# NVlabs/latentfusion

Measured on AMD Instinct MI355X. Metric: pose-optim iters/sec (reconstruct+render+backward), 16 views, 128^3 voxels, higher is better.
Workload: dtype f32

## Files before the change

### latentfusion_amd/csrc/conv_wino.hip

```cpp
#include "lf_common.h"
#ifndef WINO_ABL
#define WINO_ABL 0
#endif
#ifndef WINO_PJ_ABL
#define WINO_PJ_ABL 0
#endif
#ifndef WINO_PL
#define WINO_PL 2
#endif
#ifndef WINO_PM
#define WINO_PM 1
#endif
#ifndef WINO_PN
#define WINO_PN 3
#endif

namespace {

constexpr int TZw = 2, TYw = 8, TXw = 16;
constexpr int HZw = TZw + 2, HYw = TYw + 2, HXw = TXw + 2;
constexpr int HALOw = HZw * HYw * HXw;
constexpr int HALFw = 2 * HYw * HXw;
constexpr int HALFBw = HALFw * 64;
constexpr int NSLOTw = (HALFw * 4 + 63) / 64;
constexpr int NITw = (NSLOTw + 3) / 4;
constexpr int BUFw = 2 * HALFBw;
constexpr int PXw = 4 * 8192;
constexpr int LDSw = BUFw + PXw + 1024;

__device__ __forceinline__ void lds_barrier() {
  asm volatile("s_waitcnt lgkmcnt(0)\n\ts_barrier" ::: "memory");
}

__device__ __forceinline__ float quad_sum(float v) {
  const float a = v + __int_as_float(__builtin_amdgcn_update_dpp(0, __float_as_int(v), 0xB1, 0xF, 0xF, true));
  return a + __int_as_float(__builtin_amdgcn_update_dpp(0, __float_as_int(a), 0x4E, 0xF, 0xF, true));
}

__device__ __forceinline__ float fast_rsqrt(float x) {
  const float r = __builtin_amdgcn_rsqf(x);
  return r * (1.5f - 0.5f * x * r * r);
}
__device__ __forceinline__ float fast_rcp(float x) {
  const float r = __builtin_amdgcn_rcpf(x);
  return r * (2.f - x * r);
}

typedef float f32x2 __attribute__((ext_vector_type(2)));
__device__ __forceinline__ f32x4 pk_sub(f32x4 a, f32x4 b) {
  f32x2 lo, hi;
  const f32x2 alo = {a[0], a[1]}, ahi = {a[2], a[3]}, blo = {b[0], b[1]}, bhi = {b[2], b[3]};
  asm("v_pk_add_f32 %0, %1, %2 neg_lo:[0,1] neg_hi:[0,1]" : "=v"(lo) : "v"(alo), "v"(blo));
  asm("v_pk_add_f32 %0, %1, %2 neg_lo:[0,1] neg_hi:[0,1]" : "=v"(hi) : "v"(ahi), "v"(bhi));
  return (f32x4){lo[0], lo[1], hi[0], hi[1]};
}

__device__ __forceinline__ void pk_sub_to(f32x4& a, const f32x4 b, int gate = 0) {
  f32x2 alo = {a[0], a[1]}, ahi = {a[2], a[3]};
  const f32x2 blo = {b[0], b[1]}, bhi = {b[2], b[3]};
  asm("v_pk_add_f32 %0, %0, %1 neg_lo:[0,1] neg_hi:[0,1]" : "+v"(alo) : "v"(blo), "s"(gate));
  asm("v_pk_add_f32 %0, %0, %1 neg_lo:[0,1] neg_hi:[0,1]" : "+v"(ahi) : "v"(bhi), "s"(gate));
  a = (f32x4){alo[0], alo[1], ahi[0], ahi[1]};
}
__device__ __forceinline__ void pk_add_to(f32x4& a, const f32x4 b, int gate = 0) {
  f32x2 alo = {a[0], a[1]}, ahi = {a[2], a[3]};
  const f32x2 blo = {b[0], b[1]}, bhi = {b[2], b[3]};
  asm("v_pk_add_f32 %0, %0, %1" : "+v"(alo) : "v"(blo), "s"(gate));
  asm("v_pk_add_f32 %0, %0, %1" : "+v"(ahi) : "v"(bhi), "s"(gate));
  a = (f32x4){alo[0], alo[1], ahi[0], ahi[1]};
}
__device__ __forceinline__ void pk_fence(f32x4& a, f32x4& b) { asm("s_nop 1" : "+v"(a), "+v"(b)); }

typedef unsigned u32x4 __attribute__((ext_vector_type(4)));

typedef _Float16 f16x4 __attribute__((ext_vector_type(4)));

__device__ __forceinline__ void wino_rows_packed(f32x4 (&vx)[4][4], const float (&wt)[64], f32x4 (&Yg)[4]) {
  f32x4 m[4][4];
  f32x4 vb[8][2];
  auto operands = [&](int p) {
    const int b = p >> 1, cp = (p & 1) * 2;
#pragma unroll
    for (int h = 0; h < 2; ++h) {
      const int c = cp + h;
      if (b == 0) { pk_sub_to(vx[0][c], vx[2][c]); vb[p][h] = vx[0][c]; }
      if (b == 1) vb[p][h] = vx[1][c] + vx[2][c];
      if (b == 2) { pk_sub_to(vx[2][c], vx[1][c]); vb[p][h] = vx[2][c]; }
      if (b == 3) { pk_sub_to(vx[1][c], vx[3][c]); vb[p][h] = vx[1][c]; }
    }
    if (b != 1) pk_fence(vb[p][0], vb[p][1]);
  };
  auto row_first = [&](int b) { pk_add_to(m[b][0], m[b][1]); };
  auto row_rest = [&](int b, int gate = 0) {
    pk_add_to(m[b][0], m[b][2], gate);
    pk_sub_to(m[b][1], m[b][2], gate);
    pk_sub_to(m[b][1], m[b][3], gate);
    const f32x4 t0 = m[b][0], t1 = m[b][1];
    if (b == 0) { Yg[0] = t0; Yg[1] = t1; }
    if (b == 1) { pk_add_to(Yg[0], t0); pk_add_to(Yg[1], t1); Yg[2] = t0; Yg[3] = t1; }
    if (b == 2) { pk_add_to(Yg[0], t0); pk_add_to(Yg[1], t1); pk_sub_to(Yg[2], t0); pk_sub_to(Yg[3], t1); }
    if (b == 3) { pk_sub_to(Yg[2], t0); pk_sub_to(Yg[3], t1); }
  };
  operands(0);
#pragma unroll
  for (int p = 0; p < 8; ++p) {
    const int b = p >> 1, cp = (p & 1) * 2;
    __builtin_amdgcn_sched_barrier(0);
#pragma unroll
    for (int h = 0; h < 2; ++h)
      m[b][cp + h] = __builtin_amdgcn_mfma_f32_16x16x4f32(wt[(b * 4 + cp + h) * 4], vb[p][h][0], (f32x4){0.f, 0.f, 0.f, 0.f}, 0, 0, 0);
    __builtin_amdgcn_sched_barrier(0);
    if (p > 0) {
      if (p & 1) row_first(b);
      else row_rest(b - 1);
    }
    if (p < 7) operands(p + 1);
#pragma unroll
    for (int i = 1; i < 4; ++i)
#pragma unroll
      for (int h = 0; h < 2; ++h)
        m[b][cp + h] = __builtin_amdgcn_mfma_f32_16x16x4f32(wt[(b * 4 + cp + h) * 4 + i], vb[p][h][i], m[b][cp + h], 0, 0, 0);
    if constexpr ((WINO_ABL & 4) != 0) {
#pragma unroll
      for (int i = 0; i < 2; ++i)
#pragma unroll
        for (int h = 0; h < 2; ++h)
// ... 102 lines not shown
#pragma unroll
            for (int h = 0; h < 2; ++h) {
              const f32x4 vs = v[h] * in_scale;
              vhi[h] = __builtin_convertvector(vs, f16x4);
              const f32x4 r1 = vs - __builtin_convertvector(vhi[h], f32x4);
              vlo[h] = __builtin_convertvector(r1, f16x4);
              if constexpr ((WINO_ABL & 8) != 0)
                vl2[h] = __builtin_convertvector(r1 - __builtin_convertvector(vlo[h], f32x4), f16x4);
            }
#pragma unroll
            for (int h = 0; h < 2; ++h) m[cp + h] = __builtin_amdgcn_mfma_f32_16x16x16f16(whi[b * 4 + cp + h], vlo[h], m[cp + h], 0, 0, 0);
#pragma unroll
            for (int h = 0; h < 2; ++h) m[cp + h] = __builtin_amdgcn_mfma_f32_16x16x16f16(wlo[b * 4 + cp + h], vhi[h], m[cp + h], 0, 0, 0);
#pragma unroll
            for (int h = 0; h < 2; ++h) m[cp + h] = __builtin_amdgcn_mfma_f32_16x16x16f16(whi[b * 4 + cp + h], vhi[h], m[cp + h], 0, 0, 0);
            if constexpr ((WINO_ABL & 8) != 0) {
#pragma unroll
              for (int h = 0; h < 2; ++h) m[cp + h] = __builtin_amdgcn_mfma_f32_16x16x16f16(wlo[b * 4 + cp + h], vlo[h], m[cp + h], 0, 0, 0);
#pragma unroll
              for (int h = 0; h < 2; ++h) m[cp + h] = __builtin_amdgcn_mfma_f32_16x16x16f16(whi[b * 4 + cp + h], vl2[h], m[cp + h], 0, 0, 0);
#pragma unroll
              for (int h = 0; h < 2; ++h) m[cp + h] = __builtin_amdgcn_mfma_f32_16x16x16f16(wlo[b * 4 + cp + h], vl2[h], m[cp + h], 0, 0, 0);
            }
          }
        }
        const f32x4 t0 = m[0] + m[1] + m[2];
        const f32x4 t1 = m[1] - m[2] - m[3];
        if (b == 0) { Yg[0] = t0; Yg[1] = t1; }
        if (b == 1) { Yg[0] += t0; Yg[1] += t1; Yg[2] = t0; Yg[3] = t1; }
        if (b == 2) { Yg[0] += t0; Yg[1] += t1; Yg[2] = pk_sub(Yg[2], t0); Yg[3] = pk_sub(Yg[3], t1); }
        if (b == 3) { Yg[2] = pk_sub(Yg[2], t0); Yg[3] = pk_sub(Yg[3], t1); }
      }
    }
#pragma unroll
    for (int ji = 0; ji < 4; ++ji) *(f32x4*)(pdst + g * 4096 + (ji >> 1) * 1024 + pw[ji & 1]) = Yg[ji];
    CTS(10 + 2 * g);
  }
#undef CTS
}

struct WinoProj {
  const float* wA;
  const float* bias;
  float* zp;
  float* pnorm;
  const float* gp;
  const float* xnorm;
  float he;
  unsigned flags;
};

__device__ __forceinline__ int tr_swz(int v) { return (0x78 >> (2 * ((v >> 2) & 3))) & 3; }

template <bool SPLIT, int FUSE = 0, bool PACK = false>
__device__ __forceinline__ void conv3d_c16_wino_body(
    const float* __restrict__ x, const float* __restrict__ upack, const float* __restrict__ bias,
    float* __restrict__ y, float* __restrict__ norm_out,
    int N, int D, int H, int W, int tiles_x, int tiles_y, int tiles_z, int ntiles,
    float he, unsigned flags, float slope, float eps,
    const float* __restrict__ prev_y, const float* __restrict__ prev_norm, unsigned prev_flags,
    const float* __restrict__ amax_in, float* __restrict__ amax_out, const WinoProj pj = WinoProj()) {
  extern __shared__ __attribute__((aligned(16))) unsigned char smem[];
  unsigned char* const buf = smem;
  unsigned char* const px = smem + BUFw;

  const int tid = threadIdx.x, lane = tid & 63;
  const int fa = __builtin_amdgcn_readfirstlane(tid >> 6);
  const int n = lane & 15, kg = lane >> 4;
  const int tx = n & 7, tyb = n >> 3;

  const int nb = gridDim.x;
  const int lb = (nb % 8 == 0) ? (blockIdx.x % 8) * (nb / 8) + blockIdx.x / 8 : blockIdx.x;
  const int per = (FUSE != 0) ? ((ntiles / tiles_z + nb - 1) / nb) * tiles_z : (ntiles + nb - 1) / nb;
  const int t_begin = lb * per;
  const int t_end = min(t_begin + per, ntiles);
  if (t_begin >= t_end) return;

  const long nvox = (long)D * H * W;
  const unsigned sample_bytes = (unsigned)(nvox * 64);

  enum { F_XLO = 1, F_XHI = 2, F_YLO = 4, F_YHI = 8, F_PAD = 16, F_ALL6 = 0x2108421 };
  const int xlim = W - (tiles_x - 1) * TXw + 1, ylim = H - (tiles_y - 1) * TYw + 1;
  int hrel[NITw];
  unsigned hflags = 0;
#pragma unroll
  for (int it = 0; it < NITw; ++it) {
    const int p = (fa + 4 * it) * 64 + lane;
    const int vs = p >> 2;
    const int row = vs / HXw, rem = vs - row * HXw;
    const int xl = rem / 9, xa = rem - xl * 9;
    const int lx = 2 * xa + xl, ly = row % HYw, lz = row / HYw;
    const int sw = (((vs >> 2) & 1) << 1) | ((ly >> 1) & 1);
    const int q = (p & 3) ^ sw;
    const bool pad = vs >= HALFw;
    hrel[it] = pad ? 0 : ((lz * H + ly) * W + lx) * 64 + q * 16;
    const unsigned f = pad ? F_PAD : ((lx == 0 ? F_XLO : 0) | (lx >= xlim ? F_XHI : 0) | (ly == 0 ? F_YLO : 0) | (ly >= ylim ? F_YHI : 0));
    hflags |= f << (5 * it);
  }
  const bool last_piece_ok = ((fa + 4 * (NITw - 1)) * 64 + lane) < HALFw * 4;

  int off[8][2];
#pragma unroll
  for (int r = 0; r < 8; ++r)
#pragma unroll
    for (int dyb = 0; dyb < 2; ++dyb) {
      const int bit = ((36 * tyb + tx + r) >> 2) & 1;
      const int quarter = (kg ^ tyb ^ dyb) ^ (bit << 1);
      off[r][dyb] = (36 * tyb + tx) * 64 + quarter * 16;
    }

  int pw[2];
#pragma unroll
  for (int i = 0; i < 2; ++i) {
    const int L = (2 * tx + i) * 4 + kg;
    pw[i] = tyb * 2048 + (L ^ ((L >> 3) & 7)) * 16;
  }
  const int pr = (lane ^ ((lane >> 3) & 7)) * 16;
  const int ex = lane >> 2, eq = lane & 3;

  float wt[64];
  f16x4 whi[16], wlo[16];
  float in_scale = 1.f;
  if constexpr (!SPLIT) {
    const float* up = upack + (long)fa * 64 * 64 + lane;
#pragma unroll
    for (int k = 0; k < 64; ++k) wt[k] = up[k * 64];
  } else {
    const f16x4* up = (const f16x4*)upack + (long)fa * 16 * 2 * 64 + lane;
#pragma unroll
    for (int k = 0; k < 16; ++k) { whi[k] = up[(k * 2 + 0) * 64]; wlo[k] = up[(k * 2 + 1) * 64]; }
    if (amax_in != nullptr) {
      const float am = lf_amax_read(amax_in, lane);
      if (am > 0.f && am < 3.0e38f) {
        int ex;
        frexpf(am, &ex);
        in_scale = ldexpf(1.f, 9 - ex);
      }
    }
  }

  int cx, cy, cz, cn;
  {
    int tt = t_begin;
    cz = tt % tiles_z; tt /= tiles_z;
    cx = tt % tiles_x; tt /= tiles_x;
    cy = tt % tiles_y; cn = tt / tiles_y;
  }
  u32x4 hlo[NITw], hhi[NITw];
  auto fetch_half = [&](u32x4 (&dst)[NITw], __amdgpu_buffer_rsrc_t rs, int base, unsigned sel) {
#pragma unroll
    for (int i = 0; i < NITw; ++i) asm volatile("" : "+v"(hrel[i]));
    if (sel == 0) {
#pragma unroll
      for (int it = 0; it < NITw; ++it) dst[it] = __builtin_amdgcn_raw_buffer_load_b128(rs, base + hrel[it], 0, 0);
    } else {
      const unsigned bad = hflags & sel;
#pragma unroll
      for (int it = 0; it < NITw; ++it)
        dst[it] = __builtin_amdgcn_raw_buffer_load_b128(rs, (bad & (31u << (5 * it))) ? 0x7fffffff : base + hrel[it], 0, 0);
    }
  };
  auto halo_fetch = [&](int bx, int by, int bz, int bn, bool on, bool slide) {
    const __amdgpu_buffer_rsrc_t rs = __builtin_amdgcn_make_buffer_rsrc((void*)(x + (long)(on ? bn : 0) * nvox * 16), 0,
                                                                        on ? sample_bytes : 0u, 0x00020000);
    const int base = (((bz * TZw - 1) * H + (by * TYw - 1)) * W + (bx * TXw - 1)) * 64;
    unsigned sel = 0;
    if (bx == 0) sel |= F_XLO * F_ALL6;
    if (bx == tiles_x - 1) sel |= F_XHI * F_ALL6;
    if (by == 0) sel |= F_YLO * F_ALL6;
    if (by == tiles_y - 1) sel |= F_YHI * F_ALL6;
    if (slide) {
#pragma unroll
      for (int it = 0; it < NITw; ++it) hlo[it] = *(const u32x4*)(buf + HALFBw + (fa + 4 * it) * 1024 + lane * 16);
    } else {
      fetch_half(hlo, rs, base, sel);
    }
    fetch_half(hhi, rs, base + 2 * H * W * 64, sel);
  };
  auto halo_commit = [&]() {
#pragma unroll
    for (int it = 0; it < NITw; ++it) {
      unsigned char* dst = buf + (fa + 4 * it) * 1024 + lane * 16;
      if (it < NITw - 1 || last_piece_ok) {
        *(u32x4*)dst = hlo[it];
        *(u32x4*)(dst + HALFBw) = hhi[it];
      }
    }
  };
  const float out_scale = he / in_scale;
  const bool addmode = prev_y != nullptr && (prev_flags & LF_EPI_ADD);
  float wave_amax = 0.f;

  int pj_lo[3];
  int pj_pix[3];
  f32x4 pj_b[3];
  f32x4 pj_aw[2], pj_yp[6];
  float pj_nr[6];
  const bool pj_last_ok = n < 4;
  auto pj_column = [&](int bx, int by, int bn) {
#pragma unroll
    for (int it = 0; it < 3; ++it) {
      const int sl = (fa + 4 * it) * 16 + n;
      const int ly = sl / HXw, rem = sl - ly * HXw;
      const int xl = rem / 9, xa = rem - xl * 9;
// ... 46 lines not shown
#pragma unroll
    for (int i = 0; i < 3; ++i) asm volatile("" : "+v"(pj_lo[i]));
#pragma unroll
   for (int pl0 = 0; pl0 < 2; ++pl0) {
    f32x4 g[3];
#pragma unroll
    for (int k = 0; k < 3; ++k) g[k] = (f32x4){0.f, 0.f, 0.f, 0.f};
    if constexpr ((WINO_PJ_ABL & 2) == 0) {
#pragma unroll
    for (int i = 0; i < 4; ++i)
#pragma unroll
      for (int k = 0; k < 3; ++k)
        g[k] = __builtin_amdgcn_mfma_f32_16x16x4f32(pj_aw[pl0][i], pj_b[k][i], g[k], 0, 0, 0);
    } else {
#pragma unroll
      for (int k = 0; k < 3; ++k) g[k] = pj_b[k] + pj_aw[pl0];
    }
#pragma unroll
    for (int k = pl0 * 3; k < pl0 * 3 + 3; ++k) {
      const f32x4 yp = pj_yp[k];
      f32x4 v = g[k - pl0 * 3] * pj.he;
      if ((pj.flags & LF_EPI_PIXELNORM) && !(WINO_PJ_ABL & 2)) {
        float dot = v[0] * yp[0] + v[1] * yp[1] + v[2] * yp[2] + v[3] * yp[3];
        dot += __shfl_xor(dot, 16, 64);
        dot += __shfl_xor(dot, 32, 64);
        dot *= (1.f / 16.f);
        const float rinv = fast_rcp(pj_nr[k]);
#pragma unroll
        for (int e = 0; e < 4; ++e) v[e] = (v[e] - yp[e] * dot) * rinv;
      }
      if (pj.flags & LF_EPI_LRELU) {
#pragma unroll
        for (int e = 0; e < 4; ++e) v[e] = yp[e] > 0.f ? v[e] : v[e] * slope;
      }
      const int pl = k / 3, it = k % 3;
      if (it < 2 || fa < 3 || pj_last_ok)
        *(f32x4*)(buf + half_base + pl * (HYw * HXw * 64) + (pj_lo[it] ^ (pl * 32))) = v;
    }
   }
  };
  auto pj_slide = [&]() {
    int sbase = fa * 1024 + lane * 16;
    asm volatile("" : "+v"(sbase));
#pragma unroll
    for (int pl = 0; pl < 2; ++pl) {
      u32x4 tmp[3];
#pragma unroll
      for (int it = 0; it < 3; ++it) tmp[it] = *(const u32x4*)(buf + HALFBw + pl * (HYw * HXw * 64) + it * 4096 + sbase);
#pragma unroll
      for (int it = 0; it < 3; ++it)
        if (it < 2 || fa < 3 || lane < 16) *(u32x4*)(buf + pl * (HYw * HXw * 64) + it * 4096 + sbase) = tmp[it];
    }
  };
  f32x4 pacc[2] = {(f32x4){0.f, 0.f, 0.f, 0.f}, (f32x4){0.f, 0.f, 0.f, 0.f}};

  if constexpr (FUSE == 2) {
#pragma unroll
    for (int it = 0; it < 3; ++it) {
      const int sl = (fa + 4 * it) * 16 + n;
      const int ly = sl / HXw;
      const int q0 = kg ^ ((((sl >> 2) & 1) << 1) | ((ly >> 1) & 1));
      pj_lo[it] = sl * 64 + q0 * 16;
    }
    pj_column(cx, cy, cn);
    pj_issue(cz * TZw - 1, cn);
    pj_issue_hot(cz * TZw - 1, cn);
    pj_finish(0);
    pj_issue(cz * TZw + 1, cn);
    pj_issue_hot(cz * TZw + 1, cn);
    pj_finish(HALFBw);
  } else {
    halo_fetch(cx, cy, cz, cn, true, false);
    halo_commit();
  }
  lds_barrier();

#if WINO_ABL & 16
#define TS(k) do { if (blockIdx.x == 11 && lane == 0) ((unsigned*)norm_out)[((t - t_begin) * 4 + fa) * 16 + (k)] = (unsigned)__builtin_readcyclecounter(); } while (0)
#else
#define TS(k) do {} while (0)
#endif
  for (int t = t_begin; t < t_end; ++t) {
    TS(0);
#if WINO_ABL & 16
    unsigned* const tsp = (blockIdx.x == 11 && lane == 0) ? (unsigned*)norm_out + ((t - t_begin) * 4 + fa) * 16 : nullptr;
#else
    unsigned* const tsp = nullptr;
#endif
    switch (fa) {
      case 0: wino_compute<0, SPLIT, FUSE != 0, PACK>(buf, off, wt, whi, wlo, in_scale, px + fa * 8192, pw, tsp); break;
      case 1: wino_compute<1, SPLIT, FUSE != 0, PACK>(buf, off, wt, whi, wlo, in_scale, px + fa * 8192, pw, tsp); break;
      case 2: wino_compute<2, SPLIT, FUSE != 0, PACK>(buf, off, wt, whi, wlo, in_scale, px + fa * 8192, pw, tsp); break;
      default: wino_compute<3, SPLIT, FUSE != 0, PACK>(buf, off, wt, whi, wlo, in_scale, px + fa * 8192, pw, tsp); break;
    }
    TS(1);
    lds_barrier();
    TS(2);
    __builtin_amdgcn_s_setprio(WINO_PN);

    int nx = cx, ny = cy, nz = cz + 1, nn = cn;
    if (nz == tiles_z) { nz = 0; ++nx; }
    if (nx == tiles_x) { nx = 0; ++ny; }
    if (ny == tiles_y) { ny = 0; ++nn; }
    TS(3);

    const int bx = cx, by = cy, bz = cz, tt = cn;
    const int gx = bx * TXw + ex;
    const bool xok = gx < W;
    int voxi[4];
    bool okv[4];
#pragma unroll
    for (int j = 0; j < 2; ++j)
#pragma unroll
      for (int zo = 0; zo < 2; ++zo) {
        const int gz = bz * TZw + zo, gy = by * TYw + 2 * fa + j;
        const bool rowok = gy < H && gz < D;
        const int rowbase = rowok ? (gz * H + gy) * W : 0;
        okv[j * 2 + zo] = xok && rowok;
        voxi[j * 2 + zo] = okv[j * 2 + zo] ? rowbase + gx : 0;
      }
    f32x4 pyv[4];
    float pnv[4];
    if (prev_y != nullptr) {
      const float* pybase = prev_y + (long)tt * nvox * 16;
      const float* pnbase = prev_norm ? prev_norm + (long)tt * nvox : nullptr;
#pragma unroll
      for (int k = 0; k < 4; ++k) {
        pyv[k] = okv[k] ? *(const f32x4*)(pybase + voxi[k] * 16 + eq * 4) : (f32x4){0.f, 0.f, 0.f, 0.f};
        pnv[k] = (okv[k] && pnbase) ? pnbase[voxi[k]] : 1.f;
      }
    }
    f32x4 bv4 = (f32x4){0.f, 0.f, 0.f, 0.f};
    {
      const float* bp = bias;
      asm volatile("" : "+s"(bp));
      if (bp != nullptr) bv4 = *(const f32x4*)(bp + eq * 4);
    }
    TS(4);
    if constexpr (FUSE == 2) {
    } else {
      halo_fetch(nx, ny, nz, nn, t + 1 < t_end, nz != 0);
    }
    TS(5);

    f32x4 o[4];
#pragma unroll
    for (int j = 0; j < 2; ++j) {
      f32x4 p[4];
      if constexpr ((WINO_ABL & 2) != 0) {
        o[j * 2 + 0] = *(const f32x4*)(px + fa * 8192 + fa * 2048 + j * 1024 + pr);
        o[j * 2 + 1] = *(const f32x4*)(px + fa * 8192 + ((fa + 1) & 3) * 2048 + j * 1024 + pr);
      } else {
#pragma unroll
        for (int a2 = 0; a2 < 4; ++a2)
          p[a2] = *(const f32x4*)(px + a2 * 8192 + fa * 2048 + j * 1024 + pr);
        o[j * 2 + 0] = p[0] + p[1] + p[2];
        o[j * 2 + 1] = pk_sub(pk_sub(p[1], p[2]), p[3]);
      }
    }

    unsigned char* ybase = (unsigned char*)(y + (long)tt * nvox * 16) + eq * 16;
    float* nbase = norm_out ? norm_out + (long)tt * nvox : nullptr;
    f32x4 v[4];
    float rn[4];
#pragma unroll
    for (int k = 0; k < 4; ++k) {
      rn[k] = 1.f;
      if constexpr ((WINO_ABL & 1) != 0) { v[k] = o[k]; continue; }
      if (prev_y == nullptr || addmode) {
        float ss = 0.f;
#pragma unroll
        for (int e = 0; e < 4; ++e) {
          float u = o[k][e] * out_scale + bv4[e];
          if (addmode) u += pyv[k][e];
          if (flags & LF_EPI_LRELU) u = fmaxf(u, u * slope);
          v[k][e] = u;
          ss += u * u;
        }
        if (flags & LF_EPI_PIXELNORM) {
          const float tq = quad_sum(ss) * (1.f / 16.f) + eps;
          const float rinv = fast_rsqrt(tq);
          rn[k] = tq * rinv;
          v[k] *= rinv;
        }
      }
    }
    TS(6);
    if constexpr (FUSE != 2) halo_commit();
    TS(7);
#pragma unroll
    for (int k = 0; k < 4; ++k) {
      if (!(WINO_ABL & 1) && prev_y != nullptr && !addmode) {
        const f32x4 yp = pyv[k];
        v[k] = o[k] * out_scale;
        if (prev_flags & LF_EPI_PIXELNORM) {
          const float dot = quad_sum(v[k][0] * yp[0] + v[k][1] * yp[1] + v[k][2] * yp[2] + v[k][3] * yp[3]) * (1.f / 16.f);
          const float rinv = fast_rcp(pnv[k]);
#pragma unroll
          for (int e = 0; e < 4; ++e) v[k][e] = (v[k][e] - yp[e] * dot) * rinv;
        }
        if (prev_flags & LF_EPI_LRELU) {
#pragma unroll
          for (int e = 0; e < 4; ++e) v[k][e] = yp[e] > 0.f ? v[k][e] : v[k][e] * slope;
        }
      }
      if (okv[k]) {
        __builtin_nontemporal_store(v[k], (f32x4*)(ybase + (unsigned)(voxi[k] * 64)));
        if (!(WINO_ABL & 16) && (prev_y == nullptr || addmode) && (flags & LF_EPI_PIXELNORM) && nbase != nullptr && eq == 0) nbase[voxi[k]] = rn[k];
        if (amax_out != nullptr)
          wave_amax = fmaxf(wave_amax, fmaxf(fmaxf(fabsf(v[k][0]), fabsf(v[k][1])), fmaxf(fabsf(v[k][2]), fabsf(v[k][3]))));
      }
    }
    if constexpr (FUSE == 2) {
      __builtin_amdgcn_sched_barrier(0);
      if (t + 1 < t_end && nz != 0) {
        if constexpr ((WINO_PJ_ABL & 4) == 0) pj_slide();
        pj_issue(nz * TZw + 1, nn);
        pj_issue_hot(nz * TZw + 1, nn);
        __builtin_amdgcn_sched_barrier(0);
        pj_finish(HALFBw);
      }
      __builtin_amdgcn_sched_barrier(0);
    }
    if constexpr (FUSE == 1) {
      __builtin_amdgcn_sched_barrier(0);
      int lop = lane;
      asm volatile("" : "+v"(lop));
      const int trn = lop & 15, trk = lop >> 4;
      f32x4 pw_a[2];
#pragma unroll
      for (int zo = 0; zo < 2; ++zo)
        pw_a[zo] = *(const f32x4*)((const char*)pj.wA + (long)min(bz * TZw + zo, D - 1) * 1024 + (unsigned)(lop * 16));
#pragma unroll
      for (int k = 0; k < 4; ++k) {
        const f32x4 vz = okv[k] ? v[k] : (f32x4){0.f, 0.f, 0.f, 0.f};
        *(f32x4*)(px + (k >> 1) * 8192 + fa * 2048 + (k & 1) * 1024 + (lop >> 2) * 64 + (((lop & 3) ^ tr_swz(lop >> 2)) * 16)) = vz;
      }
      f32x4 bq[4];
#pragma unroll
      for (int k = 0; k < 4; ++k)
        bq[k] = *(const f32x4*)(px + (k >> 1) * 8192 + fa * 2048 + (k & 1) * 1024 + trn * 64 + ((trk ^ tr_swz(trn)) * 16));
#pragma unroll
      for (int zo = 0; zo < 2; ++zo)
#pragma unroll
        for (int i = 0; i < 4; ++i)
#pragma unroll
          for (int j = 0; j < 2; ++j)
            pacc[j] = __builtin_amdgcn_mfma_f32_16x16x4f32(pw_a[zo][i], bq[j * 2 + zo][i], pacc[j], 0, 0, 0);
      if (bz == tiles_z - 1) {
        f32x4 pb = (f32x4){0.f, 0.f, 0.f, 0.f};
        if (pj.bias != nullptr) pb = *(const f32x4*)(pj.bias + trk * 4);
        const int pgx = bx * TXw + trn;
#pragma unroll
        for (int j = 0; j < 2; ++j) {
          const int pgy = by * TYw + 2 * fa + j;
          float ss = 0.f;
          f32x4 u;
#pragma unroll
          for (int e = 0; e < 4; ++e) {
            float q = pacc[j][e] * pj.he + pb[e];
            if (pj.flags & LF_EPI_LRELU) q = lf_lrelu(q, slope);
            u[e] = q;
            ss += q * q;
          }
          float r = 1.f, rinv = 1.f;
          if (pj.flags & LF_EPI_PIXELNORM) {
            ss += __shfl_xor(ss, 16, 64);
            ss += __shfl_xor(ss, 32, 64);
            r = sqrtf(ss / 16.f + eps);
            rinv = 1.0f / r;
          }
          if (pgy < H && pgx < W) {
            const long pix = ((long)tt * H + pgy) * W + pgx;
            if (pj.flags & LF_EPI_PIXELNORM) { u[0] *= rinv; u[1] *= rinv; u[2] *= rinv; u[3] *= rinv; }
            *(f32x4*)(pj.zp + pix * 16 + trk * 4) = u;
            if ((pj.flags & LF_EPI_PIXELNORM) && pj.pnorm != nullptr && trk == 0) pj.pnorm[pix] = r;
          }
          pacc[j] = (f32x4){0.f, 0.f, 0.f, 0.f};
        }
      }
// ... 12 lines not shown
        pj_finish(HALFBw);
        lds_barrier();
      }
    }
  }
  if (amax_out != nullptr) {
    float m = wave_amax;
#pragma unroll
    for (int o2 = 32; o2 > 0; o2 >>= 1) m = fmaxf(m, __shfl_xor(m, o2, 64));
    lf_amax_publish(amax_out, m, lane);
  }
}

template <bool PACK>
__global__ void __launch_bounds__(256, 2) conv3d_c16_wino_kernel(
    const float* __restrict__ x, const float* __restrict__ upack, const float* __restrict__ bias,
    float* __restrict__ y, float* __restrict__ norm_out, int N, int D, int H, int W, int tiles_x, int tiles_y, int tiles_z,
    int ntiles, float he, unsigned flags, float slope, float eps, const float* __restrict__ prev_y,
    const float* __restrict__ prev_norm, unsigned prev_flags, float* __restrict__ amax_out) {
  conv3d_c16_wino_body<false, 0, PACK>(x, upack, bias, y, norm_out, N, D, H, W, tiles_x, tiles_y, tiles_z, ntiles, he, flags, slope, eps,
                              prev_y, prev_norm, prev_flags, nullptr, amax_out);
}

__global__ void __launch_bounds__(256, 2) conv3d_c16_wino_f16x3_kernel(
    const float* __restrict__ x, const float* __restrict__ upack, const float* __restrict__ bias,
    float* __restrict__ y, float* __restrict__ norm_out, int N, int D, int H, int W, int tiles_x, int tiles_y, int tiles_z,
    int ntiles, float he, unsigned flags, float slope, float eps, const float* __restrict__ prev_y,
    const float* __restrict__ prev_norm, unsigned prev_flags, const float* __restrict__ amax_in,
    float* __restrict__ amax_out) {
  conv3d_c16_wino_body<true>(x, upack, bias, y, norm_out, N, D, H, W, tiles_x, tiles_y, tiles_z, ntiles, he, flags, slope, eps,
                             prev_y, prev_norm, prev_flags, amax_in, amax_out);
}

template <bool PACK>
__global__ void __launch_bounds__(256, 2) conv3d_c16_wino_projfwd_kernel(
    const float* __restrict__ x, const float* __restrict__ upack, const float* __restrict__ bias,
    float* __restrict__ y, float* __restrict__ norm_out, int N, int D, int H, int W, int tiles_x, int tiles_y, int tiles_z,
    int ntiles, float he, unsigned flags, float slope, float eps, const float* __restrict__ prev_y,
    const float* __restrict__ prev_norm, unsigned prev_flags, WinoProj pj) {
  conv3d_c16_wino_body<false, 1, PACK>(x, upack, bias, y, norm_out, N, D, H, W, tiles_x, tiles_y, tiles_z, ntiles, he, flags, slope,
                                 eps, prev_y, prev_norm, prev_flags, nullptr, nullptr, pj);
}

template <bool PACK>
__global__ void __launch_bounds__(256, 2) conv3d_c16_wino_projbwd_kernel(
    const float* __restrict__ x, const float* __restrict__ upack, const float* __restrict__ bias,
    float* __restrict__ y, float* __restrict__ norm_out, int N, int D, int H, int W, int tiles_x, int tiles_y, int tiles_z,
    int ntiles, float he, unsigned flags, float slope, float eps, const float* __restrict__ prev_y,
    const float* __restrict__ prev_norm, unsigned prev_flags, WinoProj pj) {
  conv3d_c16_wino_body<false, 2, PACK>(x, upack, bias, y, norm_out, N, D, H, W, tiles_x, tiles_y, tiles_z, ntiles, he, flags, slope,
                                 eps, prev_y, prev_norm, prev_flags, nullptr, nullptr, pj);
}

int g_wino_pack = 1;

template <auto kernel, bool COLUMNS = false, typename... Extra>
int launch_wino(const float* x, const void* upack, const float* bias, float* y, float* norm_out, int N, int D,
                int H, int W, float he, unsigned flags, float slope, float eps, const float* prev_y, const float* prev_norm,
                unsigned prev_flags, void* stream, Extra... extra) {
  if (N <= 0 || D <= 0 || H <= 0 || W <= 0) return LF_EINVAL;
  if ((long)D * H * W * 64 >= 0x7fffffffL || !(slope > 0.f && slope < 1.f)) return LF_EINVAL;
  if (!lf_aligned16(x) || !lf_aligned16(y) || !lf_aligned16(upack) || (bias && !lf_aligned16(bias))) return LF_EALIGN;
  const bool add = prev_y != nullptr && (prev_flags & LF_EPI_ADD);
  if (add && prev_flags != LF_EPI_ADD) return LF_EINVAL;
  if (prev_y != nullptr && !add && (flags != 0 || bias != nullptr)) return LF_EINVAL;
  if ((prev_flags & LF_EPI_PIXELNORM) && prev_y != nullptr && prev_norm == nullptr) return LF_EINVAL;
  const int ptx = (W + TXw - 1) / TXw, pty = (H + TYw - 1) / TYw, ptz = (D + TZw - 1) / TZw;
  const long pt = (long)ptx * pty * ptz * N;
  if (pt > 0x7fffffffL) return LF_EINVAL;
  const int cus = lf_cu_count();
  const size_t shmem = (size_t)LDSw;
  static lf_devmask_t attr_set;
  {
    hipError_t e = lf_ensure_dyn_lds(attr_set, (const void*)kernel, (int)shmem);
    if (e != hipSuccess) return (int)e;
  }
  const long want = 2L * cus;
  const long units = COLUMNS ? pt / ptz : pt;
  const unsigned grid = (unsigned)(units < want ? units : want);
  hipLaunchKernelGGL(kernel, dim3(grid), dim3(256), shmem, (hipStream_t)stream, x, (const float*)upack, bias, y, norm_out, N, D,
                     H, W, ptx, pty, ptz, (int)pt, he, flags, slope, eps, prev_y, prev_norm, prev_flags, extra...);
  return lf_launch_status();
}

}

int lf_internal_wino_set_pack(int v) {
  const int prev = g_wino_pack;
  if (v == 0 || v == 1) g_wino_pack = v;
  return prev;
}

extern "C" size_t lf_conv3d_c16_wino_upack_floats(void) { return (size_t)4 * 16 * 4 * 64; }

extern "C" int lf_conv3d_c16_wino(const float* x, const float* upack, const float* bias, float* y, float* norm_out,
                                  int N, int D, int H, int W, float he, unsigned flags, float slope, float eps,
                                  const float* prev_y, const float* prev_norm, unsigned prev_flags,
                                  float* amax_out, void* stream) {
  lf_clear_error();
  return g_wino_pack ? launch_wino<conv3d_c16_wino_kernel<true>>(x, upack, bias, y, norm_out, N, D, H, W, he, flags, slope, eps, prev_y,
                                                                  prev_norm, prev_flags, stream, amax_out)
                     : launch_wino<conv3d_c16_wino_kernel<false>>(x, upack, bias, y, norm_out, N, D, H, W, he, flags, slope, eps, prev_y,
                                                                   prev_norm, prev_flags, stream, amax_out);
}

extern "C" size_t lf_conv3d_c16_wino_split_upack_halfs(void) { return (size_t)4 * 16 * 2 * 64 * 4; }

extern "C" int lf_conv3d_c16_wino_split(const float* x, const void* upack, const float* bias, float* y, float* norm_out,
                                        int N, int D, int H, int W, float he, unsigned flags, float slope, float eps,
                                        const float* prev_y, const float* prev_norm, unsigned prev_flags,
                                        const float* amax_in, float* amax_out, void* stream) {
  lf_clear_error();
  return launch_wino<conv3d_c16_wino_f16x3_kernel>(x, upack, bias, y, norm_out, N, D, H, W, he, flags, slope, eps, prev_y,
                     prev_norm, prev_flags, stream, amax_in, amax_out);
}

extern "C" size_t lf_conv3d_c16_wino_proj_pack_floats(int D) { return (size_t)(D > 0 ? D : 0) * 64 * 4; }

extern "C" int lf_conv3d_c16_wino_projfwd(const float* x, const float* upack, const float* bias, float* y, float* norm_out,
                                          int N, int D, int H, int W, float he, unsigned flags, float slope, float eps,
                                          const float* proj_wA, const float* proj_bias, float* zp, float* pnorm,
                                          float proj_he, unsigned proj_flags, void* stream) {
  lf_clear_error();
  if (proj_wA == nullptr || zp == nullptr) return LF_EINVAL;
  if (!lf_aligned16(proj_wA) || !lf_aligned16(zp) || (proj_bias && !lf_aligned16(proj_bias))) return LF_EALIGN;
  if ((proj_flags & ~(LF_EPI_LRELU | LF_EPI_PIXELNORM)) != 0) return LF_EINVAL;
  WinoProj pj = {proj_wA, proj_bias, zp, pnorm, nullptr, nullptr, proj_he, proj_flags};
  return g_wino_pack ? launch_wino<conv3d_c16_wino_projfwd_kernel<true>, true>(x, upack, bias, y, norm_out, N, D, H, W, he, flags, slope,
                                                                                eps, nullptr, nullptr, 0u, stream, pj)
                     : launch_wino<conv3d_c16_wino_projfwd_kernel<false>, true>(x, upack, bias, y, norm_out, N, D, H, W, he, flags, slope,
                                                                                 eps, nullptr, nullptr, 0u, stream, pj);
}

extern "C" int lf_conv3d_c16_wino_projbwd(const float* gp, const float* proj_wtA, float proj_he, const float* act,
                                          const float* act_norm, unsigned act_flags, const float* upack, float* y,
                                          int N, int D, int H, int W, float he, float slope, const float* prev_y,
                                          const float* prev_norm, unsigned prev_flags, void* stream) {
  lf_clear_error();
  if (gp == nullptr || proj_wtA == nullptr || act == nullptr) return LF_EINVAL;
  if ((act_flags & LF_EPI_PIXELNORM) && act_norm == nullptr) return LF_EINVAL;
  if ((act_flags & ~(LF_EPI_LRELU | LF_EPI_PIXELNORM)) != 0) return LF_EINVAL;
  if (!lf_aligned16(gp) || !lf_aligned16(proj_wtA) || (prev_y && !lf_aligned16(prev_y))) return LF_EALIGN;
  if (prev_y != nullptr && (prev_flags & LF_EPI_ADD)) return LF_EINVAL;
  WinoProj pj = {proj_wtA, nullptr, nullptr, nullptr, gp, act_norm, proj_he, act_flags};
  return g_wino_pack ? launch_wino<conv3d_c16_wino_projbwd_kernel<true>, true>(act, upack, nullptr, y, nullptr, N, D, H, W, he, 0u, slope,
                                                                                0.f, prev_y, prev_norm, prev_flags, stream, pj)
                     : launch_wino<conv3d_c16_wino_projbwd_kernel<false>, true>(act, upack, nullptr, y, nullptr, N, D, H, W, he, 0u, slope,
                                                                                 0.f, prev_y, prev_norm, prev_flags, stream, pj);
}
```

### latentfusion_amd/csrc/lf_common.h

```cpp
#pragma once
#include <hip/hip_runtime.h>
#include <stdint.h>
#include "../../include/lf_hip.h"
#include "../../include/lf_hip_experimental.h"

#define LF_WAVE 64

typedef float f32x4 __attribute__((ext_vector_type(4)));

static inline void lf_clear_error() { (void)hipGetLastError(); }

static inline int lf_launch_status() {
  hipError_t e = hipGetLastError();
  return (int)e;
}

static inline bool lf_aligned16(const void* p) { return (((uintptr_t)p) & 15u) == 0; }

#include <atomic>
typedef std::atomic<unsigned long long> lf_devmask_t;
static inline hipError_t lf_ensure_dyn_lds(lf_devmask_t& done, const void* fn, int bytes) {
  int dev = 0;
  if (hipGetDevice(&dev) != hipSuccess) dev = 0;
  const unsigned long long bit = 1ull << (dev & 63);
  if (done.load(std::memory_order_acquire) & bit) return hipSuccess;
  const hipError_t e = hipFuncSetAttribute(fn, hipFuncAttributeMaxDynamicSharedMemorySize, bytes);
  if (e == hipSuccess) done.fetch_or(bit, std::memory_order_release);
  return e;
}

static inline int lf_cu_count() {
  static std::atomic<int> cus[64];
  int dev = 0, v = 0;
  const bool known = hipGetDevice(&dev) == hipSuccess;
  std::atomic<int>& slot = cus[dev & 63];
  const int c = slot.load(std::memory_order_relaxed);
  if (c != 0) return c;
  const int n = (known && hipDeviceGetAttribute(&v, hipDeviceAttributeMultiprocessorCount, dev) == hipSuccess && v > 0) ? v : 256;
  slot.store(n, std::memory_order_relaxed);
  return n;
}

__device__ __forceinline__ float lf_wave_sum(float v) {
#pragma unroll
  for (int o = 32; o > 0; o >>= 1) v += __shfl_xor(v, o, 64);
  return v;
}

#define LF_AMAX_SLOTS 64
#define LF_AMAX_STRIDE 32
static_assert(LF_AMAX_FLOATS == LF_AMAX_SLOTS * LF_AMAX_STRIDE, "lf_hip.h: LF_AMAX_FLOATS");

__device__ __forceinline__ void lf_amax_publish(float* base, float wave_max, int lane) {
  if (lane == 0 && wave_max > 0.f)
    atomicMax((unsigned int*)(base + (blockIdx.x % LF_AMAX_SLOTS) * LF_AMAX_STRIDE), __float_as_uint(wave_max));
}

__device__ __forceinline__ float lf_amax_read(const float* base, int lane) {
  float m = base[(lane % LF_AMAX_SLOTS) * LF_AMAX_STRIDE];
#pragma unroll
  for (int o = 32; o > 0; o >>= 1) m = fmaxf(m, __shfl_xor(m, o, 64));
  return m;
}

__device__ __forceinline__ float lf_lrelu(float v, float slope) { return v > 0.f ? v : v * slope; }

int lf_internal_ring_bf16_set_wgs(int v);
int lf_internal_wino_set_pack(int v);
int lf_internal_fused_set_cfg(int v);
int lf_internal_splat_set_variant(int v);
int lf_internal_splat_set_chunk_cap(int v);
```

### latentfusion_amd/csrc/resample.hip

```cpp
#include "resample_map.h"

namespace {

typedef unsigned u32x4_t __attribute__((ext_vector_type(4)));

struct Tap {
  int x0, y0, z0, x1, y1, z1;
  float tx, ty, tz;
  float mx, my, mz;
};

__device__ __forceinline__ float lattice01(int i, int size, float step) {
  return (i < size / 2) ? step * (float)i : 1.f - step * (float)(size - 1 - i);
}


template <int KIND>
__device__ __forceinline__ void eval_grid(const float* __restrict__ cf, int x, int y, int z,
                                          int W, int H, int D, Steps st, float& gx, float& gy, float& gz,
                                          float& a, float& b, float& k) {
  a = lattice01(x, W, st.w);
  b = lattice01(y, H, st.h);
  k = lattice01(z, D, st.d);
  if (KIND == LF_MAP_O2C) {
// ... 462 lines not shown
  if (((uintptr_t)vol_idx & 3) != 0) return LF_EALIGN;
  BwdCoefPlan p;
  if (int e = bwd_coef_plan(gout, vol, scratch_bytes, N, part_n, D, H, W, C, p)) return e;
  const long bstride = p.nvox * C;
  hipStream_t s = (hipStream_t)stream;
  float* partial = (float*)scratch;
  if (g_resample_variant >= 2 && p.vec && C == 16 && p.vpb >= 64 && p.nvox * 64 < 0xffffffffL) {
    if (p.vpb >= 256)
      hipLaunchKernelGGL((resample_bwd_coef_c16_dedup_indexed_kernel<2, 1, true>), p.grid, dim3(256), 0, s, gout, vol, bstride, vol_idx, vol_n, coef, partial, p.nblk, p.vpb, p.bt, D, H, W, p.st);
    else
      hipLaunchKernelGGL((resample_bwd_coef_c16_indexed_kernel<8, 1>), p.grid, dim3(256), 0, s, gout, vol, bstride, vol_idx, vol_n, coef, partial, p.nblk, p.vpb, p.bt, D, H, W, p.st);
  } else if (p.vec) {
    hipLaunchKernelGGL((resample_bwd_coef_indexed_kernel<4>), p.grid, dim3(256), 0, s, gout, vol, bstride, vol_idx, vol_n, coef, partial, p.nblk, p.vpb, p.bt, N, D, H, W, C, p.lpv, p.st);
  } else {
    hipLaunchKernelGGL((resample_bwd_coef_indexed_kernel<1>), p.grid, dim3(256), 0, s, gout, vol, bstride, vol_idx, vol_n, coef, partial, p.nblk, p.vpb, p.bt, N, D, H, W, C, p.lpv, p.st);
  }
  return bwd_coef_finish(partial, p.nblk, gcoef, N, s);
}

extern "C" int lf_resample3d_bwd_vol(const float* gout, const float* coef, int kind, float* gvol, int vol_n,
                                     int N, int D, int H, int W, int C, void* stream) {
  lf_clear_error();
  if (N <= 0 || D <= 0 || H <= 0 || W <= 0 || C <= 0) return LF_EINVAL;
  if (vol_n != 1 && vol_n != N) return LF_EINVAL;
  const long bstride = vol_n == 1 ? 0 : (long)D * H * W * C;
  const long items = (long)D * H * W * C;
  dim3 grid((unsigned)min((items + 255) / 256, (long)65535 * 16), N), block(256);
  hipStream_t s = (hipStream_t)stream;
  if (kind == LF_MAP_O2C)
    hipLaunchKernelGGL((resample_bwd_vol_kernel<LF_MAP_O2C>), grid, block, 0, s, gout, coef, gvol, bstride, N, D, H, W, C, make_steps(D, H, W));
  else if (kind == LF_MAP_C2O)
    hipLaunchKernelGGL((resample_bwd_vol_kernel<LF_MAP_C2O>), grid, block, 0, s, gout, coef, gvol, bstride, N, D, H, W, C, make_steps(D, H, W));
  else
    return LF_EINVAL;
  return lf_launch_status();
}

#ifdef STAGE_TS
extern "C" int lf_debug_stage_ts(void* dst) {
  return (int)hipMemcpyFromSymbol(dst, HIP_SYMBOL(g_stage_ts), sizeof(unsigned long long) * 256 * 16, 0, hipMemcpyDeviceToHost);
}
#endif

extern "C" int lf_set_tuning(int key, int value) {
  if (key == 1) {
    const int prev = g_resample_variant;
    if (value >= 1 && value <= 5) g_resample_variant = value;
    return prev;
  }
  if (key == 4) return lf_internal_splat_set_variant(value);
  if (key == 6) return lf_internal_splat_set_chunk_cap(value);
  if (key == 3) return lf_internal_fused_set_cfg(value);
  if (key == 7) return lf_internal_wino_set_pack(value);
  if (key == 5) return lf_internal_ring_bf16_set_wgs(value);
  if (key == 2) {
    const int prev = g_bwd_coef_variant;
    if (value >= 1 && value <= 11) g_bwd_coef_variant = value;
    return prev;
  }
  return LF_EINVAL;
}

extern "C" int lf_resample3d_fwd_io(const void* vol, int vol_n, const float* coef, int kind, void* out,
                                    int N, int D, int H, int W, int io, void* stream) {
  lf_clear_error();
  if (N <= 0 || D <= 0 || H <= 0 || W <= 0 || io < 0 || io > 3) return LF_EINVAL;
  if ((vol_n != 1 && vol_n != N) || (kind != LF_MAP_O2C && kind != LF_MAP_C2O)) return LF_EINVAL;
  if (!lf_aligned16(vol) || !lf_aligned16(out)) return LF_EALIGN;
  if ((long)D * H * W * 64 >= 0xffffffffL) return LF_EINVAL;
  const long bstride = vol_n == 1 ? 0 : (long)D * H * W * 16;
  const int nbz4 = (D + 3) >> 2;
  if ((long)nbz4 * N > 65535 || ((H + 3) >> 2) > 65535) return LF_EINVAL;
  dim3 g4((unsigned)((W + 3) >> 2), (unsigned)((H + 3) >> 2), (unsigned)(nbz4 * N)), block(256);
  const Steps st = make_steps(D, H, W);
  typedef void (*kern_t)(const float*, long, const float*, float*, int, int, int, int, Steps);
  static const kern_t kerns[2][4] = {
      {resample_fwd_c16_kernel<LF_MAP_O2C, 0>, resample_fwd_c16_kernel<LF_MAP_O2C, 1>, resample_fwd_c16_kernel<LF_MAP_O2C, 2>, resample_fwd_c16_kernel<LF_MAP_O2C, 3>},
      {resample_fwd_c16_kernel<LF_MAP_C2O, 0>, resample_fwd_c16_kernel<LF_MAP_C2O, 1>, resample_fwd_c16_kernel<LF_MAP_C2O, 2>, resample_fwd_c16_kernel<LF_MAP_C2O, 3>}};
  hipLaunchKernelGGL(kerns[kind == LF_MAP_O2C ? 0 : 1][io], g4, block, 0, (hipStream_t)stream, (const float*)vol, bstride, coef, (float*)out, D, H, W, nbz4, st);
  return lf_launch_status();
}
```

Baseline: 193.1.

## Add specialized Winograd conv kernels for fixed epilogue forms

Adds template-specialized Winograd conv3d kernels for three common epilogue configurations: forward bias+lrelu+pixelnorm, dgrad through a previous lrelu+pixelnorm, and plain dgrad. A host-side dispatcher picks a form from the arguments. Each form folds flag and null checks into compile-time constants and uses a dedicated epilogue built on DPP quad reductions, rsq/rcp with Newton refinement, and hoisted bias loads. By default (OPT=1) it also drops some register-pinning asm barriers. The goal is less runtime branching and fewer epilogue instructions, at the cost of more kernel instantiations, different scheduling and slightly different rounding.

```diff
diff --git a/latentfusion_amd/csrc/conv_wino.hip b/latentfusion_amd/csrc/conv_wino.hip
--- a/latentfusion_amd/csrc/conv_wino.hip
+++ b/latentfusion_amd/csrc/conv_wino.hip
@@ -72,6 +72,49 @@
 __device__ __forceinline__ void pk_fence(f32x4& a, f32x4& b) { asm("s_nop 1" : "+v"(a), "+v"(b)); }
 
 typedef unsigned u32x4 __attribute__((ext_vector_type(4)));
+
+__device__ __forceinline__ float quad_sum_pinned(float v) {
+  float a, b;
+  asm("s_nop 4\n\tv_add_f32_dpp %0, %1, %1 quad_perm:[1,0,3,2] row_mask:0xf bank_mask:0xf bound_ctrl:1" : "=v"(a) : "v"(v));
+  asm("s_nop 4\n\tv_add_f32_dpp %0, %1, %1 quad_perm:[2,3,0,1] row_mask:0xf bank_mask:0xf bound_ctrl:1" : "=v"(b) : "v"(a));
+  return b;
+}
+__device__ __forceinline__ void wino_epi_fwd_block(const f32x4 o, const f32x4 b, float scale, float slope, float eps,
+                                                   f32x4& v, float& rn) {
+#pragma clang fp contract(off)
+  f32x4 u;
+#pragma unroll
+  for (int e = 0; e < 4; ++e) {
+    const float t = __builtin_fmaf(scale, o[e], b[e]);
+    u[e] = fmaxf(t, t * slope);
+  }
+  const float ss = __builtin_fmaf(u[3], u[3], __builtin_fmaf(u[2], u[2], __builtin_fmaf(u[0], u[0], u[1] * u[1])));
+  const float tq = __builtin_fmaf(quad_sum_pinned(ss), 1.f / 16.f, eps);
+  const float r = __builtin_amdgcn_rsqf(tq);
+  const float rinv = r * __builtin_fmaf(r, (-0.5f * tq) * r, 1.5f);
+  rn = tq * rinv;
+  v = u * rinv;
+}
+__device__ __forceinline__ f32x4 wino_epi_dgrad_prev(const f32x4 o, const f32x4 yp, float pn, float scale, float slope) {
+#pragma clang fp contract(off)
+  f32x4 v = o * scale;
+  const float dot = quad_sum_pinned(((v[0] * yp[0] + v[1] * yp[1]) + v[2] * yp[2]) + v[3] * yp[3]) * (1.f / 16.f);
+  const float r = __builtin_amdgcn_rcpf(pn);
+  const float rinv = r * (2.f - pn * r);
+  v[0] = __builtin_fmaf(-yp[0], dot, v[0]) * rinv;
+  v[1] = __builtin_fmaf(-yp[1], dot, v[1]) * rinv;
+  v[2] = (v[2] - yp[2] * dot) * rinv;
+  v[3] = (v[3] - yp[3] * dot) * rinv;
+#pragma unroll
+  for (int e = 0; e < 4; ++e) v[e] = yp[e] > 0.f ? v[e] : v[e] * slope;
+  return v;
+}
+__device__ __forceinline__ f32x4 wino_epi_dgrad_plain(const f32x4 o, float scale) {
+  f32x4 v;
+#pragma unroll
+  for (int e = 0; e < 4; ++e) v[e] = __builtin_fmaf(scale, o[e], 0.f);
+  return v;
+}
 
 typedef _Float16 f16x4 __attribute__((ext_vector_type(4)));
 
@@ -280,7 +323,13 @@
 
 __device__ __forceinline__ int tr_swz(int v) { return (0x78 >> (2 * ((v >> 2) & 3))) & 3; }
 
-template <bool SPLIT, int FUSE = 0, bool PACK = false>
+enum : int {
+  WF_GENERIC = 0,
+  WF_FWD_BLOCK = 1,
+  WF_DGRAD_PREV = 2,
+  WF_DGRAD_PLAIN = 3,
+};
+template <bool SPLIT, int FUSE = 0, bool PACK = false, int FORM = WF_GENERIC, int OPT = 0>
 __device__ __forceinline__ void conv3d_c16_wino_body(
     const float* __restrict__ x, const float* __restrict__ upack, const float* __restrict__ bias,
     float* __restrict__ y, float* __restrict__ norm_out,
@@ -288,6 +337,20 @@
     float he, unsigned flags, float slope, float eps,
     const float* __restrict__ prev_y, const float* __restrict__ prev_norm, unsigned prev_flags,
     const float* __restrict__ amax_in, float* __restrict__ amax_out, const WinoProj pj = WinoProj()) {
+  static_assert(FORM == WF_GENERIC || (!SPLIT && FUSE != 2 && PACK), "fixed forms: the packed all-fp32 kernels only");
+  static_assert(OPT == 0 || OPT == 1, "");
+  static_assert(FORM != WF_GENERIC || OPT == 0, "the generic kernel stays as it is");
+  constexpr bool HAS_BIAS = FORM == WF_FWD_BLOCK;
+  if constexpr (FORM == WF_FWD_BLOCK) {
+    flags = LF_EPI_LRELU | LF_EPI_PIXELNORM;
+    prev_y = nullptr; prev_norm = nullptr; prev_flags = 0u; amax_out = nullptr;
+  } else if constexpr (FORM == WF_DGRAD_PREV) {
+    flags = 0u; prev_flags = LF_EPI_LRELU | LF_EPI_PIXELNORM;
+    bias = nullptr; norm_out = nullptr; amax_out = nullptr;
+  } else if constexpr (FORM == WF_DGRAD_PLAIN) {
+    flags = 0u; prev_flags = 0u;
+    bias = nullptr; norm_out = nullptr; prev_y = nullptr; prev_norm = nullptr; amax_out = nullptr;
+  }
   extern __shared__ __attribute__((aligned(16))) unsigned char smem[];
   unsigned char* const buf = smem;
   unsigned char* const px = smem + BUFw;
@@ -376,8 +439,10 @@
   }
   u32x4 hlo[NITw], hhi[NITw];
   auto fetch_half = [&](u32x4 (&dst)[NITw], __amdgpu_buffer_rsrc_t rs, int base, unsigned sel) {
-#pragma unroll
-    for (int i = 0; i < NITw; ++i) asm volatile("" : "+v"(hrel[i]));
+    if constexpr (!(OPT & 1)) {
+#pragma unroll
+      for (int i = 0; i < NITw; ++i) asm volatile("" : "+v"(hrel[i]));
+    }
     if (sel == 0) {
 #pragma unroll
       for (int it = 0; it < NITw; ++it) dst[it] = __builtin_amdgcn_raw_buffer_load_b128(rs, base + hrel[it], 0, 0);
@@ -530,6 +595,8 @@
         if (it < 2 || fa < 3 || lane < 16) *(u32x4*)(buf + pl * (HYw * HXw * 64) + it * 4096 + sbase) = tmp[it];
     }
   };
+  f32x4 bv_res = (f32x4){0.f, 0.f, 0.f, 0.f};
+  if constexpr (HAS_BIAS && (OPT & 1)) bv_res = *(const f32x4*)(bias + eq * 4);
   f32x4 pacc[2] = {(f32x4){0.f, 0.f, 0.f, 0.f}, (f32x4){0.f, 0.f, 0.f, 0.f}};
 
   if constexpr (FUSE == 2) {
@@ -601,18 +668,24 @@
     float pnv[4];
     if (prev_y != nullptr) {
       const float* pybase = prev_y + (long)tt * nvox * 16;
-      const float* pnbase = prev_norm ? prev_norm + (long)tt * nvox : nullptr;
+      const float* pnbase = (FORM == WF_DGRAD_PREV || prev_norm) ? prev_norm + (long)tt * nvox : nullptr;
 #pragma unroll
       for (int k = 0; k < 4; ++k) {
         pyv[k] = okv[k] ? *(const f32x4*)(pybase + voxi[k] * 16 + eq * 4) : (f32x4){0.f, 0.f, 0.f, 0.f};
-        pnv[k] = (okv[k] && pnbase) ? pnbase[voxi[k]] : 1.f;
+        pnv[k] = (okv[k] && (FORM == WF_DGRAD_PREV || pnbase)) ? pnbase[voxi[k]] : 1.f;
       }
     }
     f32x4 bv4 = (f32x4){0.f, 0.f, 0.f, 0.f};
-    {
+    if constexpr (FORM == WF_GENERIC) {
       const float* bp = bias;
       asm volatile("" : "+s"(bp));
       if (bp != nullptr) bv4 = *(const f32x4*)(bp + eq * 4);
+    } else if constexpr (HAS_BIAS && (OPT & 1)) {
+      bv4 = bv_res;
+    } else if constexpr (HAS_BIAS) {
+      const float* bp = bias;
+      asm volatile("" : "+s"(bp));
+      bv4 = *(const f32x4*)(bp + eq * 4);
     }
     TS(4);
     if constexpr (FUSE == 2) {
@@ -638,14 +711,18 @@
     }
 
     unsigned char* ybase = (unsigned char*)(y + (long)tt * nvox * 16) + eq * 16;
-    float* nbase = norm_out ? norm_out + (long)tt * nvox : nullptr;
+    float* nbase = (FORM == WF_FWD_BLOCK || norm_out) ? norm_out + (long)tt * nvox : nullptr;
     f32x4 v[4];
     float rn[4];
 #pragma unroll
     for (int k = 0; k < 4; ++k) {
       rn[k] = 1.f;
       if constexpr ((WINO_ABL & 1) != 0) { v[k] = o[k]; continue; }
-      if (prev_y == nullptr || addmode) {
+      if constexpr (FORM == WF_FWD_BLOCK) {
+        wino_epi_fwd_block(o[k], bv4, out_scale, slope, eps, v[k], rn[k]);
+      } else if constexpr (FORM == WF_DGRAD_PLAIN) {
+        v[k] = wino_epi_dgrad_plain(o[k], out_scale);
+      } else if (prev_y == nullptr || addmode) {
         float ss = 0.f;
 #pragma unroll
         for (int e = 0; e < 4; ++e) {
@@ -668,7 +745,9 @@
     TS(7);
 #pragma unroll
     for (int k = 0; k < 4; ++k) {
-      if (!(WINO_ABL & 1) && prev_y != nullptr && !addmode) {
+      if constexpr (FORM == WF_DGRAD_PREV) {
+        if (!(WINO_ABL & 1)) v[k] = wino_epi_dgrad_prev(o[k], pyv[k], pnv[k], out_scale, slope);
+      } else if (!(WINO_ABL & 1) && prev_y != nullptr && !addmode) {
         const f32x4 yp = pyv[k];
         v[k] = o[k] * out_scale;
         if (prev_flags & LF_EPI_PIXELNORM) {
@@ -684,7 +763,7 @@
       }
       if (okv[k]) {
         __builtin_nontemporal_store(v[k], (f32x4*)(ybase + (unsigned)(voxi[k] * 64)));
-        if (!(WINO_ABL & 16) && (prev_y == nullptr || addmode) && (flags & LF_EPI_PIXELNORM) && nbase != nullptr && eq == 0) nbase[voxi[k]] = rn[k];
+        if (!(WINO_ABL & 16) && (prev_y == nullptr || addmode) && (flags & LF_EPI_PIXELNORM) && (FORM == WF_FWD_BLOCK || nbase != nullptr) && eq == 0) nbase[voxi[k]] = rn[k];
         if (amax_out != nullptr)
           wave_amax = fmaxf(wave_amax, fmaxf(fmaxf(fabsf(v[k][0]), fabsf(v[k][1])), fmaxf(fabsf(v[k][2]), fabsf(v[k][3]))));
       }
@@ -703,7 +782,7 @@
     if constexpr (FUSE == 1) {
       __builtin_amdgcn_sched_barrier(0);
       int lop = lane;
-      asm volatile("" : "+v"(lop));
+      if constexpr (!(OPT & 1)) asm volatile("" : "+v"(lop));
       const int trn = lop & 15, trk = lop >> 4;
       f32x4 pw_a[2];
 #pragma unroll
@@ -822,7 +901,38 @@
                                  eps, prev_y, prev_norm, prev_flags, nullptr, nullptr, pj);
 }
 
+template <int FORM, int OPT>
+__global__ void __launch_bounds__(256, 2) conv3d_c16_wino_form_kernel(
+    const float* __restrict__ x, const float* __restrict__ upack, const float* __restrict__ bias,
+    float* __restrict__ y, float* __restrict__ norm_out, int N, int D, int H, int W, int tiles_x, int tiles_y, int tiles_z,
+    int ntiles, float he, unsigned flags, float slope, float eps, const float* __restrict__ prev_y,
+    const float* __restrict__ prev_norm, unsigned prev_flags, float* __restrict__ amax_out) {
+  conv3d_c16_wino_body<false, 0, true, FORM, OPT>(x, upack, bias, y, norm_out, N, D, H, W, tiles_x, tiles_y, tiles_z, ntiles, he, flags,
+                                                 slope, eps, prev_y, prev_norm, prev_flags, nullptr, amax_out);
+}
+
+template <int FORM, int OPT>
+__global__ void __launch_bounds__(256, 2) conv3d_c16_wino_projfwd_form_kernel(
+    const float* __restrict__ x, const float* __restrict__ upack, const float* __restrict__ bias,
+    float* __restrict__ y, float* __restrict__ norm_out, int N, int D, int H, int W, int tiles_x, int tiles_y, int tiles_z,
+    int ntiles, float he, unsigned flags, float slope, float eps, const float* __restrict__ prev_y,
+    const float* __restrict__ prev_norm, unsigned prev_flags, WinoProj pj) {
+  conv3d_c16_wino_body<false, 1, true, FORM, OPT>(x, upack, bias, y, norm_out, N, D, H, W, tiles_x, tiles_y, tiles_z, ntiles, he, flags,
+                                                 slope, eps, prev_y, prev_norm, prev_flags, nullptr, nullptr, pj);
+}
+
 int g_wino_pack = 1;
+int g_wino_forms = 1;
+
+int wino_form_of(const float* bias, const float* norm_out, unsigned flags, const float* prev_y, const float* prev_norm,
+                 unsigned prev_flags, const float* amax_out) {
+  const unsigned full = LF_EPI_LRELU | LF_EPI_PIXELNORM;
+  if (!g_wino_pack || !g_wino_forms || amax_out != nullptr) return WF_GENERIC;
+  if (flags == full && bias != nullptr && norm_out != nullptr && prev_y == nullptr) return WF_FWD_BLOCK;
+  if (flags == 0u && bias == nullptr && prev_y != nullptr && prev_norm != nullptr && prev_flags == full) return WF_DGRAD_PREV;
+  if (flags == 0u && bias == nullptr && prev_y == nullptr) return WF_DGRAD_PLAIN;
+  return WF_GENERIC;
+}
 
 template <auto kernel, bool COLUMNS = false, typename... Extra>
 int launch_wino(const float* x, const void* upack, const float* bias, float* y, float* norm_out, int N, int D,
@@ -860,6 +970,11 @@
   if (v == 0 || v == 1) g_wino_pack = v;
   return prev;
 }
+int lf_internal_wino_set_forms(int v) {
+  const int prev = g_wino_forms;
+  if (v >= 0 && v <= 2) g_wino_forms = v;
+  return prev;
+}
 
 extern "C" size_t lf_conv3d_c16_wino_upack_floats(void) { return (size_t)4 * 16 * 4 * 64; }
 
@@ -868,6 +983,18 @@
                                   const float* prev_y, const float* prev_norm, unsigned prev_flags,
                                   float* amax_out, void* stream) {
   lf_clear_error();
+#define LF_WINO_FORM(F, O) \
+  launch_wino<conv3d_c16_wino_form_kernel<F, O>>(x, upack, bias, y, norm_out, N, D, H, W, he, flags, slope, eps, prev_y, prev_norm, \
+                                                 prev_flags, stream, amax_out)
+#define LF_WINO_OPTS(F) (g_wino_forms == 2 ? LF_WINO_FORM(F, 0) : LF_WINO_FORM(F, 1))
+  switch (wino_form_of(bias, norm_out, flags, prev_y, prev_norm, prev_flags, amax_out)) {
+    case WF_FWD_BLOCK: return LF_WINO_OPTS(WF_FWD_BLOCK);
+    case WF_DGRAD_PREV: return LF_WINO_OPTS(WF_DGRAD_PREV);
+    case WF_DGRAD_PLAIN: return LF_WINO_OPTS(WF_DGRAD_PLAIN);
+    default: break;
+  }
+#undef LF_WINO_OPTS
+#undef LF_WINO_FORM
   return g_wino_pack ? launch_wino<conv3d_c16_wino_kernel<true>>(x, upack, bias, y, norm_out, N, D, H, W, he, flags, slope, eps, prev_y,
                                                                   prev_norm, prev_flags, stream, amax_out)
                      : launch_wino<conv3d_c16_wino_kernel<false>>(x, upack, bias, y, norm_out, N, D, H, W, he, flags, slope, eps, prev_y,
@@ -896,6 +1023,13 @@
   if (!lf_aligned16(proj_wA) || !lf_aligned16(zp) || (proj_bias && !lf_aligned16(proj_bias))) return LF_EALIGN;
   if ((proj_flags & ~(LF_EPI_LRELU | LF_EPI_PIXELNORM)) != 0) return LF_EINVAL;
   WinoProj pj = {proj_wA, proj_bias, zp, pnorm, nullptr, nullptr, proj_he, proj_flags};
+  if (wino_form_of(bias, norm_out, flags, nullptr, nullptr, 0u, nullptr) == WF_FWD_BLOCK) {
+#define LF_WINO_FORM(O) \
+  launch_wino<conv3d_c16_wino_projfwd_form_kernel<WF_FWD_BLOCK, O>, true>(x, upack, bias, y, norm_out, N, D, H, W, he, flags, slope, eps, \
+                                                                          nullptr, nullptr, 0u, stream, pj)
+    return g_wino_forms == 2 ? LF_WINO_FORM(0) : LF_WINO_FORM(1);
+#undef LF_WINO_FORM
+  }
   return g_wino_pack ? launch_wino<conv3d_c16_wino_projfwd_kernel<true>, true>(x, upack, bias, y, norm_out, N, D, H, W, he, flags, slope,
                                                                                 eps, nullptr, nullptr, 0u, stream, pj)
                      : launch_wino<conv3d_c16_wino_projfwd_kernel<false>, true>(x, upack, bias, y, norm_out, N, D, H, W, he, flags, slope,
diff --git a/latentfusion_amd/csrc/lf_common.h b/latentfusion_amd/csrc/lf_common.h
--- a/latentfusion_amd/csrc/lf_common.h
+++ b/latentfusion_amd/csrc/lf_common.h
@@ -67,6 +67,7 @@
 
 int lf_internal_ring_bf16_set_wgs(int v);
 int lf_internal_wino_set_pack(int v);
+int lf_internal_wino_set_forms(int v);
 int lf_internal_fused_set_cfg(int v);
 int lf_internal_splat_set_variant(int v);
 int lf_internal_splat_set_chunk_cap(int v);
diff --git a/latentfusion_amd/csrc/resample.hip b/latentfusion_amd/csrc/resample.hip
--- a/latentfusion_amd/csrc/resample.hip
+++ b/latentfusion_amd/csrc/resample.hip
@@ -538,6 +538,7 @@
   if (key == 6) return lf_internal_splat_set_chunk_cap(value);
   if (key == 3) return lf_internal_fused_set_cfg(value);
   if (key == 7) return lf_internal_wino_set_pack(value);
+  if (key == 8) return lf_internal_wino_set_forms(value);
   if (key == 5) return lf_internal_ring_bf16_set_wgs(value);
   if (key == 2) {
     const int prev = g_bwd_coef_variant;
```

New measurement: 196.8, median of 6. 1.9% higher.
